# JosefAlbers/Phi-3-Vision-MLX

Hardware: AMD Instinct MI355X
Metric: decode tokens/sec through generate()'s loop (reference-defined; bare graph replays: device_rate) + prefill ms, Phi-3-Vision bf16 1-image VQA (higher is better)
Workload: dtype bf16; 1 GPU; Phi-3-Vision single 336x336 image VQA (BASELINE configs[1]); 17 crops, 2509 image tokens + 22 text tokens, prompt 2531, B=1 per GPU, greedy, EOS suppressed; parallelism=batch-sharded replicas x1, batch_per_gpu=1, tiny=False

## Files before the change

### phi-3-vision-mlx_amd/csrc/p3v_common.h

```cpp
#pragma once
#include <hip/hip_runtime.h>
#include <stdint.h>

#include "../../include/p3v.h"

typedef uint16_t bf16_t;
typedef __attribute__((ext_vector_type(8))) __bf16 bf16x8_t;
typedef __attribute__((ext_vector_type(4))) float f32x4_t;
typedef __attribute__((ext_vector_type(16))) float f32x16_t;
typedef __attribute__((ext_vector_type(4))) uint32_t u32x4_t;
typedef __attribute__((ext_vector_type(2))) uint32_t u32x2_t;

#define P3V_WAVE 64
#define P3V_MAX_DEVICES 64

#define P3V_CHECK_LAUNCH()                                   \
  do {                                                       \
    hipError_t e_ = hipGetLastError();                       \
    if (e_ != hipSuccess) return P3V_ERR_LAUNCH;             \
  } while (0)

__device__ __forceinline__ float bf16_to_f32(bf16_t u) { return __uint_as_float(((uint32_t)u) << 16); }

typedef __attribute__((ext_vector_type(2))) __bf16 bf16x2_t;
// ... 46 lines not shown
__device__ __forceinline__ float rows_sum(float v) {
  float a, b;
  rows_swap32(v, a, b); v = a + b;
  rows_swap16(v, a, b); return a + b;
}

#define P3V_DPP_F32(v, ctrl) __builtin_bit_cast(float, __builtin_amdgcn_update_dpp(0, __builtin_bit_cast(int, v), ctrl, 0xf, 0xf, true))
__device__ __forceinline__ float wave_sum(float v) {
  v += P3V_DPP_F32(v, 0xB1);
  v += P3V_DPP_F32(v, 0x4E);
  v += P3V_DPP_F32(v, 0x124);
  v += P3V_DPP_F32(v, 0x128);
  return rows_sum(v);
}
__device__ __forceinline__ float wave_max(float v) {
  v = fmaxf(v, P3V_DPP_F32(v, 0xB1));
  v = fmaxf(v, P3V_DPP_F32(v, 0x4E));
  v = fmaxf(v, P3V_DPP_F32(v, 0x124));
  v = fmaxf(v, P3V_DPP_F32(v, 0x128));
  return rows_max(v);
}

__device__ __forceinline__ float block_sum(float v, float* red) {
  v = wave_sum(v);
  const int w = threadIdx.x >> 6, nw = blockDim.x >> 6;
  __syncthreads();
  if ((threadIdx.x & 63) == 0) red[w] = v;
  __syncthreads();
  float t = 0.f;
  for (int i = 0; i < nw; ++i) t += red[i];
  return t;
}
__device__ __forceinline__ float block_max(float v, float* red) {
  v = wave_max(v);
  const int w = threadIdx.x >> 6, nw = blockDim.x >> 6;
  __syncthreads();
  if ((threadIdx.x & 63) == 0) red[w] = v;
  __syncthreads();
  float t = -INFINITY;
  for (int i = 0; i < nw; ++i) t = fmaxf(t, red[i]);
  return t;
}

static inline int p3v_cdiv(long a, long b) { return (int)((a + b - 1) / b); }
static inline int p3v_gemv_wpw(int waves, int n_cu, int forced) {
  if (forced == 3 || forced == 4) return forced;
  const float w3 = (float)p3v_cdiv(p3v_cdiv(waves, 3), n_cu) * 3.f * n_cu / (float)waves;
  const float w4 = (float)p3v_cdiv(p3v_cdiv(waves, 4), n_cu) * 4.f * n_cu / (float)waves;
  return w3 < w4 - 0.05f ? 3 : 4;
}

struct P3vTuning {
  int gemm_big_rows;
  int gemm_no_splitk, gemm_splitk_max_m, gemm_splitk_max_s, gemm_splitk_wgs, gemm_128, gemm_persistent;
  int gemm_rows;
  int gemm_no_skinny, gemm_skinny_max_m, gemm_skinny_s, gemm_skinny_tm128;
  int gemm_no_qkv_fuse;
  int gemm_f8_narrow;
  int attn_no_dma, attn_old, attn_pp, attn_il, attn_il_waves, combine_g, kvq_old, q8_old;
  int attn_fo_map_q8;
  int attn_fo_map;
  int gemv_no_mfma, gemv_no_mfma8, gemv_wpc, gemv8_wgs, gemv_variant, gemv_rows, gemv8_min, gemv_mfma8, gemv_f8_wpc, gemv_q4_wpc, gemv_wpw, gemv_q4_rows_wgs, gemv_q4_rows8;
};
const P3vTuning& p3v_tuning();
```

### phi-3-vision-mlx_amd/csrc/p3v_gemm.hip

```cpp
#include <stdlib.h>
#include <string.h>


#include "p3v_gemm_qkv.h"

#define P3V_EPI_QKV 100

#define BM 128
#define BN 128
#define BK 64
#define TILE_BYTES (BM * BK * 2)
#define GEMM_LDS (4 * TILE_BYTES)

typedef const __attribute__((address_space(1))) void* gptr_t;
typedef __attribute__((address_space(3))) void* lptr_t;

struct GemmP {
  const bf16_t* A; const bf16_t* W; void* out; const bf16_t* bias; const void* resid; const bf16_t* pos;
  int M, N, K, lda, ldw, ldo, ppi;
  int kslice;
  QkvP q;
};

__device__ __forceinline__ float gelu_erf(float x) { return 0.5f * x * (1.f + erff(x * 0.70710678118654752f)); }
// ... 204 lines not shown
#pragma unroll
    for (int jp = 0; jp < 2; ++jp) {
      uint32_t pk[2][2];
#pragma unroll
      for (int jj = 0; jj < 2; ++jj) {
        const int j = 2 * jp + jj;
        float v[4];
#pragma unroll
        for (int r = 0; r < 4; ++r) {
          v[r] = acc[i][j][r] + bias[j][r];
          if (EPI == P3V_EPI_BIAS_QGELU) v[r] = v[r] * p3v_sigmoid(1.702f * v[r]);
          else if (EPI == P3V_EPI_BIAS_GELU) v[r] = gelu_erf(v[r]);
        }
        pk[jj][0] = pack_bf16x2(v[0], v[1]), pk[jj][1] = pack_bf16x2(v[2], v[3]);
      }
      u32x4_t w;
#pragma unroll
      for (int k = 0; k < 2; ++k) {
        auto sw = __builtin_amdgcn_permlane16_swap(pk[0][k], pk[1][k], false, false);
        w[k] = sw[0], w[2 + k] = sw[1];
      }
      const int n = n0 + wc * 64 + (2 * jp + (fq & 1)) * 16 + (fq >> 1) * 8;
      if (m < p.M && n < p.N) {
        const size_t o = (size_t)m * p.ldo + n;
        if (EPI == P3V_EPI_RESID_BF16) {
          const u32x4_t rw = *(const u32x4_t*)((const bf16_t*)p.resid + o);
#pragma unroll
          for (int k = 0; k < 4; ++k) w[k] = pack_bf16x2(bf16lo(rw[k]) + bf16lo(w[k]), bf16hi(rw[k]) + bf16hi(w[k]));
        }
        *(u32x4_t*)((bf16_t*)p.out + o) = w;
      }
    }
  }
}

template <int EPI, int ORD>
static int launch_gemm_v(const GemmP& p, hipStream_t s) {
  static bool attr_set = false;
  if (!attr_set) {
    if (hipFuncSetAttribute((const void*)k_gemm<EPI, ORD>, hipFuncAttributeMaxDynamicSharedMemorySize, GEMM_LDS) != hipSuccess)
      return P3V_ERR_HIP;
    attr_set = true;
  }
  const int n_tile = EPI == P3V_EPI_SILU_MUL ? BN / 2 : BN;
  dim3 grid(p3v_cdiv(p.N, n_tile), p3v_cdiv(p.M, BM), p.kslice ? p.K / p.kslice : 1);
  hipLaunchKernelGGL((k_gemm<EPI, ORD>), grid, dim3(256), GEMM_LDS, s, p);
  P3V_CHECK_LAUNCH();
  return P3V_OK;
}

template <int EPI>
static int launch_gemm(const GemmP& p, hipStream_t s) { return launch_gemm_v<EPI, 0>(p, s); }

int p3v_gemm256_try(const p3v_gemm_args_t* a, hipStream_t s);
static int gemm128(const p3v_gemm_args_t* a, hipStream_t s);

static int gemm_big_rows(const p3v_gemm_args_t* a) {
  const int n_big = a->epilogue == P3V_EPI_SILU_MUL ? 128 : 256, n_small = n_big / 2;
  if (a->M < 1024 || a->N % n_big || a->epilogue == P3V_EPI_PATCH) return 0;
  if (const int force = p3v_tuning().gemm_big_rows; force >= 0) return min(force / 256 * 256, a->M);
  const int mt = p3v_cdiv(a->M, 256), nt_big = a->N / n_big, nt_small = p3v_cdiv(a->N, n_small);
  const float big_round = a->K >= 2048 ? 1.0f : 1.0f + 0.25f * (2048 - a->K) / 1024.f;
  float best = 1e30f;
  int best_rows = 0;
  for (int ms = 0; ms <= mt; ++ms) {
    const int rows_big = min(ms * 256, a->M), rows_small = a->M - rows_big;
    const long big = (long)ms * nt_big, small = (long)p3v_cdiv(rows_small, 128) * nt_small;
    float c = (float)((big + 255) / 256) * big_round;
    if (small) {
      const long full = small / 512, rest = small % 512;
      c += 0.675f * full + (rest == 0 ? 0.f : rest <= 256 ? 0.42f : 0.675f);
    }
    if (big && small) c += 0.04f;
    if (c < best - 1e-4f) { best = c; best_rows = rows_big; }
  }
  return best_rows;
}

template <int EPI>
__global__ void __launch_bounds__(256) k_splitk_reduce(const float* __restrict__ part, void* __restrict__ out, const void* __restrict__ resid,
                                                       int M, int N, int ldp, int ldo, int S) {
  constexpr bool SILU = EPI == P3V_EPI_SILU_MUL;
  const int per_row = N / 8;
  const long i = (long)blockIdx.x * 256 + threadIdx.x;
  if (i >= (long)M * per_row) return;
  const int m = (int)(i / per_row), n = (int)(i - (long)m * per_row) * 8;
  float v[8] = {0, 0, 0, 0, 0, 0, 0, 0}, u[8] = {0, 0, 0, 0, 0, 0, 0, 0};
  for (int z = 0; z < S; ++z) {
    const float* pr = part + ((size_t)z * M + m) * ldp + n;
    const float4 a0 = *(const float4*)pr, a1 = *(const float4*)(pr + 4);
    v[0] += a0.x; v[1] += a0.y; v[2] += a0.z; v[3] += a0.w; v[4] += a1.x; v[5] += a1.y; v[6] += a1.z; v[7] += a1.w;
    if (SILU) {
      const float4 b0 = *(const float4*)(pr + N), b1 = *(const float4*)(pr + N + 4);
      u[0] += b0.x; u[1] += b0.y; u[2] += b0.z; u[3] += b0.w; u[4] += b1.x; u[5] += b1.y; u[6] += b1.z; u[7] += b1.w;
    }
  }
  const size_t o = (size_t)m * ldo + n;
  if (SILU) {
#pragma unroll
    for (int e = 0; e < 8; ++e) {
      const float g = bf16_round(v[e]), up = bf16_round(u[e]);
      v[e] = bf16_round(g * bf16_round(1.f / (1.f + __expf(-g)))) * up;
    }
  } else if (EPI == P3V_EPI_RESID_BF16) {
    float r[8];
    load8_bf16((const bf16_t*)resid + o, r);
#pragma unroll
    for (int e = 0; e < 8; ++e) v[e] = r[e] + bf16_round(v[e]);
  }
  store8_bf16((bf16_t*)out + o, v);
}

__global__ void __launch_bounds__(384) k_splitk_reduce_norm(const float* __restrict__ part, bf16_t* __restrict__ out, const bf16_t* __restrict__ resid,
                                                            const u32x4_t* __restrict__ norm_w, u32x4_t* __restrict__ normed, int M, int N,
                                                            int ldo, int S, float inv_h, float eps) {
  __shared__ float ps[6 * 4][64];
  __shared__ float r_sh;
  const int row = blockIdx.x, c = threadIdx.x, lane = c & 63, wv = c >> 6, chunks = N / 8;
  u32x4_t v = {0u, 0u, 0u, 0u}, g = {0u, 0u, 0u, 0u};
  if (c < chunks) {
    float acc[8] = {0, 0, 0, 0, 0, 0, 0, 0};
    for (int z = 0; z < S; ++z) {
      const float* pr = part + ((size_t)z * M + row) * N + c * 8;
      const float4 a0 = *(const float4*)pr, a1 = *(const float4*)(pr + 4);
      acc[0] += a0.x; acc[1] += a0.y; acc[2] += a0.z; acc[3] += a0.w; acc[4] += a1.x; acc[5] += a1.y; acc[6] += a1.z; acc[7] += a1.w;
    }
    const size_t o = (size_t)row * ldo + c * 8;
    float r[8];
    load8_bf16(resid + o, r);
// ... 76 lines not shown
}

int p3v_splitk_reduce(const float* part, const p3v_gemm_args_t* a, int S, hipStream_t s) {
  const bool silu = a->epilogue == P3V_EPI_SILU_MUL;
  const int w_rows = silu ? 2 * a->N : a->N;
  const long items = (long)a->M * (a->N / 8);
  const dim3 grid((unsigned)p3v_cdiv(items, 256));
  if (silu) hipLaunchKernelGGL(k_splitk_reduce<P3V_EPI_SILU_MUL>, grid, dim3(256), 0, s, part, a->out, a->resid, a->M, a->N, w_rows, a->ldo, S);
  else if (a->epilogue == P3V_EPI_RESID_BF16)
    hipLaunchKernelGGL(k_splitk_reduce<P3V_EPI_RESID_BF16>, grid, dim3(256), 0, s, part, a->out, a->resid, a->M, a->N, w_rows, a->ldo, S);
  else hipLaunchKernelGGL(k_splitk_reduce<P3V_EPI_NONE>, grid, dim3(256), 0, s, part, a->out, a->resid, a->M, a->N, w_rows, a->ldo, S);
  P3V_CHECK_LAUNCH();
  return P3V_OK;
}

static int gemm_splitk(const p3v_gemm_args_t* a, hipStream_t s) {
  const bool silu = a->epilogue == P3V_EPI_SILU_MUL;
  const int S = splitk_slices(a->M, a->N, a->K, a->epilogue);
  if (S == 1) return P3V_ERR_UNSUPPORTED;
  const int w_rows = silu ? 2 * a->N : a->N;
  if (!a->ws || a->ws_bytes < (int64_t)S * a->M * w_rows * 4) return P3V_ERR_UNSUPPORTED;
  if ((uintptr_t)a->ws & 15) return P3V_ERR_ARG;
  float* part = (float*)a->ws;
  GemmP p = {a->A, a->W, part, nullptr, nullptr, nullptr, a->M, w_rows, a->K, a->lda, a->ldw, w_rows, 0, a->K / S, {}};
  const int rc = launch_gemm<P3V_EPI_F32>(p, s);
  if (rc != P3V_OK) return rc;
  return p3v_splitk_reduce(part, a, S, s);
}

extern "C" int p3v_gemm(const p3v_gemm_args_t* a, void* stream) {
  if (!a || !a->A || !a->W || !a->out) return P3V_ERR_ARG;
  if (a->M < 0 || a->N <= 0 || a->K <= 0 || a->K % BK || a->N % 8 || a->ldo % 8) return P3V_ERR_ARG;
  if (a->lda < a->K || a->ldw < a->K || a->lda % 8 || a->ldw % 8) return P3V_ERR_ARG;
  if (((uintptr_t)a->A | (uintptr_t)a->W | (uintptr_t)a->out | (uintptr_t)a->resid | (uintptr_t)a->bias | (uintptr_t)a->pos) & 15)
    return P3V_ERR_ARG;
  if ((a->epilogue == P3V_EPI_BIAS_RESID_F32 || a->epilogue == P3V_EPI_RESID_BF16) && !a->resid) return P3V_ERR_ARG;
  if (a->epilogue == P3V_EPI_PATCH && (!a->pos || a->patches_per_img <= 0)) return P3V_ERR_ARG;
  if (a->epilogue < 0 || a->epilogue > P3V_EPI_F32) return P3V_ERR_ARG;
  if (a->M == 0) return P3V_OK;
  {
    const size_t w_rows = (size_t)a->N * (a->epilogue == P3V_EPI_SILU_MUL ? 2 : 1);
    if ((size_t)a->M * a->lda * 2 >= (1ull << 32) || w_rows * a->ldw * 2 >= (1ull << 32)) return P3V_ERR_UNSUPPORTED;
  }
  hipStream_t s = (hipStream_t)stream;
  if (!a->bias) {
    const int rc = p3v_gemm_skinny_try(a, s);
    if (rc != P3V_ERR_UNSUPPORTED) return rc;
  }
  {
    const int rc = gemm_splitk(a, s);
    if (rc != P3V_ERR_UNSUPPORTED) return rc;
  }
  const bool big_tiles = !p3v_tuning().gemm_128;
  const int rows_big = big_tiles ? gemm_big_rows(a) : 0;
  if (rows_big > 0) {
    p3v_gemm_args_t top = *a;
    top.M = rows_big;
    const int rc = p3v_gemm256_try(&top, s);
    if (rc == P3V_OK && rows_big < a->M) {
      const bool f32_out = a->epilogue == P3V_EPI_BIAS_RESID_F32 || a->epilogue == P3V_EPI_F32;
      const size_t out_row = (size_t)a->ldo * (f32_out ? 4 : 2);
      p3v_gemm_args_t rest = *a;
      rest.M = a->M - rows_big;
      rest.A = a->A + (size_t)rows_big * a->lda;
      rest.out = (char*)a->out + rows_big * out_row;
      if (a->resid) rest.resid = (const char*)a->resid + rows_big * out_row;
      return gemm128(&rest, s);
    }
    if (rc != P3V_ERR_UNSUPPORTED) return rc;
  }
  return gemm128(a, s);
}

static int gemm128(const p3v_gemm_args_t* a, hipStream_t s) {
  const GemmP p = {a->A, a->W, a->out, a->bias, a->resid, a->pos,
                   a->M, a->N, a->K, a->lda, a->ldw, a->ldo, a->patches_per_img, 0, {}};
  switch (a->epilogue) {
    case P3V_EPI_NONE: return launch_gemm<P3V_EPI_NONE>(p, s);
    case P3V_EPI_BIAS: return launch_gemm<P3V_EPI_BIAS>(p, s);
    case P3V_EPI_BIAS_QGELU: return launch_gemm<P3V_EPI_BIAS_QGELU>(p, s);
    case P3V_EPI_BIAS_GELU: return launch_gemm<P3V_EPI_BIAS_GELU>(p, s);
    case P3V_EPI_BIAS_RESID_F32: return launch_gemm<P3V_EPI_BIAS_RESID_F32>(p, s);
    case P3V_EPI_RESID_BF16: return launch_gemm<P3V_EPI_RESID_BF16>(p, s);
    case P3V_EPI_SILU_MUL: return launch_gemm<P3V_EPI_SILU_MUL>(p, s);
    case P3V_EPI_PATCH: return launch_gemm<P3V_EPI_PATCH>(p, s);
    case P3V_EPI_F32: return launch_gemm<P3V_EPI_F32>(p, s);
    default: return P3V_ERR_ARG;
  }
}

int p3v_gemm256_qkv(const p3v_gemm_args_t* a, const QkvP& q, hipStream_t s);
int p3v_gemm_skinny_qkv(const p3v_gemm_args_t* a, const QkvP& q, hipStream_t s);

extern "C" int p3v_gemm_qkv(const p3v_gemm_args_t* a, const p3v_qkv_split_t* sp, void* stream) {
  if (!a || !sp || !a->A || !a->W || !sp->q_out || !sp->k_dst || !sp->v_dst || (!sp->cos_t) != (!sp->sin_t)) return P3V_ERR_ARG;
  if (a->epilogue != P3V_EPI_NONE && a->epilogue != P3V_EPI_BIAS) return P3V_ERR_ARG;
  if (a->epilogue == P3V_EPI_BIAS && !a->bias) return P3V_ERR_ARG;
  const int nh = sp->n_heads, nkv = sp->n_kv, hd = sp->hd, half = hd / 2;
  if (sp->B <= 0 || sp->L <= 0 || nh <= 0 || nkv <= 0 || hd <= 0 || sp->tab_div <= 0 || !(sp->q_scale > 0.f)) return P3V_ERR_ARG;
  if (a->M != sp->B * sp->L || a->N != (nh + 2 * nkv) * hd || a->K % BK || a->lda < a->K || a->ldw < a->K || a->lda % 8 || a->ldw % 8) return P3V_ERR_ARG;
  if (((uintptr_t)a->A | (uintptr_t)a->W | (uintptr_t)a->bias | (uintptr_t)sp->q_out | (uintptr_t)sp->k_dst | (uintptr_t)sp->v_dst |
       (uintptr_t)sp->cos_t | (uintptr_t)sp->sin_t) & 15)
    return P3V_ERR_ARG;
  const int dpos0 = sp->dst_off_is_past ? sp->past : 0;
  if (hd % 32 || half % 16 || dpos0 % 8 || sp->dst_t % 8 || p3v_tuning().gemm_no_qkv_fuse) return P3V_ERR_UNSUPPORTED;
  if ((size_t)a->M * a->lda * 2 >= (1ull << 32) || (size_t)a->N * a->ldw * 2 >= (1ull << 32)) return P3V_ERR_UNSUPPORTED;
  hipStream_t s = (hipStream_t)stream;
  QkvP q = {sp->cos_t, sp->sin_t, sp->q_out, sp->k_dst, sp->v_dst, sp->L, nh, nkv, hd, sp->past, dpos0, sp->dst_t, sp->tab_t, sp->tab_div, 0,
            sp->q_scale};
  if (a->M < 1024) return p3v_gemm_skinny_qkv(a, q, s);
  if ((nh * hd) % BN || (nkv * hd) % BN || p3v_tuning().gemm_128) return P3V_ERR_UNSUPPORTED;
// ... 18 lines not shown
```

### phi-3-vision-mlx_amd/csrc/p3v_gemm256.hip

```cpp
#include <stdlib.h>

#include "p3v_gemm256_epi.h"

#define BUF_BYTES (4 * HALF_BYTES)
#define GEMM256_LDS (2 * BUF_BYTES)

struct Tile256 {
  int m0, n0; int a_off[2][2], b_off[2][2]; __amdgpu_buffer_rsrc_t rs_a;
  int swapped, is_k, row0;
};

#ifdef P3V_G256_DEBUG
__device__ unsigned long long p3v_g256dbg[8 * 64 * 8];
#define G_S(k) do { __builtin_amdgcn_sched_barrier(0); asm volatile("s_memtime %0" : "=s"(g_s[k])); __builtin_amdgcn_sched_barrier(0); } while (0)
#define G_FLUSH(it) do { if (blockIdx.x == P3V_G256_DEBUG && (threadIdx.x & 63) == 0 && (it) < 64) { for (int k_ = 0; k_ < 8; ++k_) p3v_g256dbg[((threadIdx.x >> 6) * 64 + (it)) * 8 + k_] = g_s[k_]; } } while (0)
extern "C" int p3v_g256dbg_read(unsigned long long* out) {
  return hipMemcpyFromSymbol(out, HIP_SYMBOL(p3v_g256dbg), sizeof(unsigned long long) * 8 * 64 * 8) == hipSuccess ? 0 : -1;
}
#else
#define G_S(k) do { } while (0)
#define G_FLUSH(it) do { } while (0)
#endif
template <int EPI, int SCHED = 0x50, int ORDER = 0>
__global__ void __launch_bounds__(512, 1) k_gemm256(Gemm256P p) {
  constexpr bool SILU = EPI == P3V_EPI_SILU_MUL, QKV = EPI == P3V_EPI_QKV;
  extern __shared__ __attribute__((aligned(16))) unsigned char smem[];
  const int tid = threadIdx.x, lane = tid & 63, wave = __builtin_amdgcn_readfirstlane(tid >> 6);
  const int wr = wave >> 2, wc = wave & 3;
  constexpr int n_out_tile = SILU ? TN / 2 : TN;
  const int gx = (p.N + n_out_tile - 1) / n_out_tile, gy = (p.M + TM - 1) / TM, nwg = gx * gy;
  const int nq_t = QKV ? p.q.nh * p.q.hd / TN : 0, nk_t = QKV ? p.q.nkv * p.q.hd / TN : 0;

  using Tile = Tile256;
  const int srow = tid >> 3, schunk = tid & 7;
  auto make_tile = [&](int wid, Tile& t) {
    const int q = nwg >> 3, r = nwg & 7, xcd = wid & 7, loc = wid >> 3;
    const int id = (xcd < r ? xcd * (q + 1) : r * (q + 1) + (xcd - r) * q) + loc;
    constexpr int BAND = 4;
    const int band = id / (BAND * gx), in_band = id % (BAND * gx);
    const int rows = min(BAND, gy - band * BAND);
    const int m_t = band * BAND + in_band % rows, n_t = in_band / rows;
    t.m0 = m_t * TM, t.n0 = n_t * n_out_tile;
    t.swapped = t.is_k = t.row0 = 0;
    if (QKV) {
      t.swapped = n_t >= nq_t + nk_t;
      t.is_k = !t.swapped && n_t >= nq_t;
      t.row0 = t.swapped ? (p.q.nh + p.q.nkv) * p.q.hd : t.is_k ? p.q.nh * p.q.hd : 0;
      t.n0 = (n_t - (t.swapped ? nq_t + nk_t : t.is_k ? nq_t : 0)) * TN;
    }
#pragma unroll
    for (int h = 0; h < 2; ++h)
#pragma unroll
      for (int qq = 0; qq < 2; ++qq) {
        const int rr = h * 128 + qq * 64 + srow;
        const int sw = (schunk ^ (rr & 7)) * 8;
        const int ar = min(t.m0 + rr, p.M - 1) - t.m0;
        int br;
        if (SILU) {
          const int wcol = rr >> 6, ni = (rr & 63) >> 4, c = rr & 15;
          br = min(t.n0 + wcol * 32 + (ni & 1) * 16 + c, p.N - 1) + (ni >> 1) * p.N;
        } else if (QKV) {
          br = qkv_pair_row(p.q, t.row0, t.n0 >> 1, rr);
        } else {
          br = min(t.n0 + rr, p.N - 1);
        }
        if (QKV && t.swapped) {
          t.a_off[h][qq] = (rr * p.ldw + sw) * 2;
          t.b_off[h][qq] = (int)(((unsigned)(t.m0 + ar) * (unsigned)p.lda + (unsigned)sw) * 2u);
        } else {
          t.a_off[h][qq] = (ar * p.lda + sw) * 2;
          t.b_off[h][qq] = (int)(((unsigned)br * (unsigned)p.ldw + (unsigned)sw) * 2u);
        }
      }
    t.rs_a = QKV && t.swapped ? __builtin_amdgcn_make_buffer_rsrc((void*)(p.W + (size_t)(t.row0 + t.n0) * p.ldw), 0, 0xffffffff, 0x00020000)
                              : __builtin_amdgcn_make_buffer_rsrc((void*)(p.A + (size_t)t.m0 * p.lda), 0, 0xffffffff, 0x00020000);
  };
  const __amdgpu_buffer_rsrc_t rs_w = __builtin_amdgcn_make_buffer_rsrc((void*)p.W, 0, 0xffffffff, 0x00020000);
  const __amdgpu_buffer_rsrc_t rs_x = __builtin_amdgcn_make_buffer_rsrc((void*)p.A, 0, 0xffffffff, 0x00020000);
  auto dma_half = [&](const Tile& t, int which, int kt, int buf) {
    unsigned char* base = smem + buf * BUF_BYTES + which * HALF_BYTES + wave * 1024;
    const int h = which & 1;
#pragma unroll
    for (int q = 0; q < 2; ++q) {
      const __amdgpu_buffer_rsrc_t rs = which < 2 ? t.rs_a : (QKV && t.swapped) ? rs_x : rs_w;
      const int vo = which < 2 ? t.a_off[h][q] : t.b_off[h][q];
      __builtin_amdgcn_raw_ptr_buffer_load_lds(rs, (lptr_t)(base + q * 8192), 16, vo, kt * (TK * 2), 0, 0);
    }
  };

  const int frow = lane & 15, fchunk = lane >> 4;
  const int nk = p.K / TK;
  int wid = blockIdx.x;
  if (wid >= nwg) return;
  Tile cur_t;
  make_tile(wid, cur_t);
#pragma unroll
  for (int w4 = 0; w4 < 4; ++w4) dma_half(cur_t, w4, 0, 0);
  int gk = 0;
  bool landed = false;
  for (;;) {
  const int m0 = cur_t.m0, n0 = cur_t.n0;
  const bool has_next = wid + (int)gridDim.x < nwg;
  f32x4_t acc[8][4];
#pragma unroll
  for (int i = 0; i < 8; ++i)
#pragma unroll
    for (int j = 0; j < 4; ++j) acc[i][j] = (f32x4_t){0.f, 0.f, 0.f, 0.f};

#ifdef P3V_G256_DEBUG
  unsigned long long g_s[8] = {0, 0, 0, 0, 0, 0, 0, 0};
#endif
  for (int kt = 0; kt < nk; ++kt, ++gk) {
    G_S(0);
    if (!(kt == 0 && landed)) asm volatile("s_waitcnt vmcnt(0)" ::: "memory");
    G_S(1);
    __builtin_amdgcn_s_barrier();
    G_S(2);
    const bool last = kt + 1 == nk;
    const bool more = !last || has_next;
    const int nb = (gk + 1) & 1;
    const unsigned char* ta = smem + (gk & 1) * BUF_BYTES + wr * HALF_BYTES;
    const unsigned char* tb = smem + (gk & 1) * BUF_BYTES + (2 + (wc >> 1)) * HALF_BYTES + (wc & 1) * 64 * 128;
    bf16x8_t af[4][2], af1[4][2], bf0[2][2], bf1[2][2];
    auto read_a_to = [&](int sub, bf16x8_t (&dst)[4][2]) {
#pragma unroll
      for (int i = 0; i < 4; ++i)
#pragma unroll
        for (int kk = 0; kk < 2; ++kk) {
          const int r = sub * 64 + i * 16 + frow;
          dst[i][kk] = *(const bf16x8_t*)(ta + r * 128 + (((kk * 4 + fchunk) ^ (r & 7)) << 4));
        }
    };
    auto read_a = [&](int sub) { read_a_to(sub, af); };
    auto read_b = [&](int sub, bf16x8_t (&bf)[2][2]) {
#pragma unroll
      for (int j = 0; j < 2; ++j)
#pragma unroll
        for (int kk = 0; kk < 2; ++kk) {
          const int r = sub * 32 + j * 16 + frow;
          bf[j][kk] = *(const bf16x8_t*)(tb + r * 128 + (((kk * 4 + fchunk) ^ (r & 7)) << 4));
        }
    };
    auto quad_from = [&](int asub, int bsub, bf16x8_t (&a)[4][2], bf16x8_t (&bf)[2][2]) {
      __builtin_amdgcn_s_setprio(1);
#pragma unroll
      for (int kk = 0; kk < 2; ++kk)
#pragma unroll
        for (int i = 0; i < 4; ++i)
#pragma unroll
          for (int j = 0; j < 2; ++j)
            acc[asub * 4 + i][bsub * 2 + j] =
                __builtin_amdgcn_mfma_f32_16x16x32_bf16(bf[j][kk], a[i][kk], acc[asub * 4 + i][bsub * 2 + j], 0, 0, 0);
      __builtin_amdgcn_s_setprio(0);
    };
    auto quad = [&](int asub, int bsub, bf16x8_t (&bf)[2][2]) { quad_from(asub, bsub, af, bf); };
    auto dma_phase = [&](int ph) {
      if (more) {
#pragma unroll
        for (int h = 0; h < 4; ++h)
          if (((SCHED >> (2 * h)) & 3) == ph) {
            if (!last) dma_half(cur_t, h, kt + 1, nb);
            else {
              Tile nt;
              make_tile(wid + gridDim.x, nt);
              dma_half(nt, h, 0, nb);
            }
          }
      }
    };
    if (ORDER == 2) {
      read_b(0, bf0);
      read_a_to(0, af);
      dma_phase(0);
      read_b(1, bf1);
      __builtin_amdgcn_sched_barrier(0);
      G_S(3);
      quad_from(0, 0, af, bf0);
      __builtin_amdgcn_sched_barrier(0);
      G_S(4);
      read_a_to(1, af1);
      dma_phase(1);
      __builtin_amdgcn_sched_barrier(0);
      G_S(5);
      quad_from(0, 1, af, bf1);
      __builtin_amdgcn_sched_barrier(0);
      G_S(6);
      quad_from(1, 1, af1, bf1);
      quad_from(1, 0, af1, bf0);
      G_S(7);
      G_FLUSH(kt);
      continue;
    }
    if (ORDER == 0) dma_phase(0);
    read_b(0, bf0);
    read_a(0);
    if (ORDER == 1) dma_phase(0);
    quad(0, 0, bf0);
    if (ORDER == 0) dma_phase(1);
    read_b(1, bf1);
    if (ORDER == 1) dma_phase(1);
    quad(0, 1, bf1);
    if (ORDER == 0) dma_phase(2);
    read_a(1);
    if (ORDER == 1) dma_phase(2);
    quad(1, 1, bf1);
    dma_phase(3);
    quad(1, 0, bf0);
  }

  if (has_next) {
    asm volatile("s_waitcnt vmcnt(0)" ::: "memory");
    landed = true;
  }
  if constexpr (QKV) {
    if (!cur_t.swapped) qkv_epilogue_rot<8>(p.q, acc, p.bias, cur_t.is_k, cur_t.row0, (n0 >> 1) + wc * 32, m0 + wr * 128, p.M, lane);
    else qkv_epilogue_vt<8>(p.q, acc, p.bias ? p.bias + cur_t.row0 : nullptr, n0 + wr * 128, m0 + wc * 64, p.M, lane);
  } else {
    gemm256_epilogue<EPI>(p, acc, m0, n0, wr, wc, lane);
  }
  if (!has_next) break;
  wid += gridDim.x;
  make_tile(wid, cur_t);
  }
}

template <int EPI, int SCHED, int ORDER>
static int launch_gemm256_v(const Gemm256P& p, hipStream_t s) {
  static bool attr_set = false;
  if (!attr_set) {
    if (hipFuncSetAttribute((const void*)k_gemm256<EPI, SCHED, ORDER>, hipFuncAttributeMaxDynamicSharedMemorySize, GEMM256_LDS) != hipSuccess)
      return P3V_ERR_HIP;
    attr_set = true;
  }
  const int n_tile = EPI == P3V_EPI_SILU_MUL ? TN / 2 : TN;
  static int n_cu = 0;
  if (!n_cu) {
    int dev = 0;
    hipDeviceProp_t pr;
    if (hipGetDevice(&dev) != hipSuccess || hipGetDeviceProperties(&pr, dev) != hipSuccess) return P3V_ERR_HIP;
    n_cu = pr.multiProcessorCount / 8 * 8;
  }
  const int tiles = p3v_cdiv(p.N, n_tile) * p3v_cdiv(p.M, TM);
  const int persist = p3v_tuning().gemm_persistent;
  dim3 grid(persist ? min(tiles, n_cu) : tiles);
  hipLaunchKernelGGL((k_gemm256<EPI, SCHED, ORDER>), grid, dim3(512), GEMM256_LDS, s, p);
  P3V_CHECK_LAUNCH();
  return P3V_OK;
}

template <int EPI>
static int launch_gemm256(const Gemm256P& p, hipStream_t s) { return launch_gemm256_v<EPI, 0x50, 2>(p, s); }

int p3v_gemm256_qkv(const p3v_gemm_args_t* a, const QkvP& q, hipStream_t s) {
  if (a->N % TN || a->K % TK || (q.nh * q.hd) % TN || (q.nkv * q.hd) % TN) return P3V_ERR_UNSUPPORTED;
  if ((size_t)a->N * a->ldw * 2 >= ((size_t)1 << 32) || (size_t)a->M * a->lda * 2 >= ((size_t)1 << 32)) return P3V_ERR_UNSUPPORTED;
  const Gemm256P p = {a->A, a->W, nullptr, a->bias, nullptr, a->M, a->N, a->K, a->lda, a->ldw, 0, q};
  return launch_gemm256<P3V_EPI_QKV>(p, s);
}

int p3v_gemm256_try(const p3v_gemm_args_t* a, hipStream_t s) {
  const int n_tile = a->epilogue == P3V_EPI_SILU_MUL ? TN / 2 : TN;
  if (a->N % n_tile || a->K % TK || a->epilogue == P3V_EPI_PATCH) return P3V_ERR_UNSUPPORTED;
  const size_t w_rows = (size_t)a->N * (a->epilogue == P3V_EPI_SILU_MUL ? 2 : 1);
  if (w_rows * a->ldw * 2 >= ((size_t)1 << 32) || (size_t)256 * a->lda * 2 >= ((size_t)1 << 31)) return P3V_ERR_UNSUPPORTED;
  const Gemm256P p = {a->A, a->W, a->out, a->bias, a->resid, a->M, a->N, a->K, a->lda, a->ldw, a->ldo, {}};
  switch (a->epilogue) {
    case P3V_EPI_NONE: return launch_gemm256<P3V_EPI_NONE>(p, s);
    case P3V_EPI_BIAS: return launch_gemm256<P3V_EPI_BIAS>(p, s);
    case P3V_EPI_BIAS_QGELU: return launch_gemm256<P3V_EPI_BIAS_QGELU>(p, s);
    case P3V_EPI_BIAS_GELU: return launch_gemm256<P3V_EPI_BIAS_GELU>(p, s);
    case P3V_EPI_BIAS_RESID_F32: return launch_gemm256<P3V_EPI_BIAS_RESID_F32>(p, s);
    case P3V_EPI_RESID_BF16: return launch_gemm256<P3V_EPI_RESID_BF16>(p, s);
    case P3V_EPI_SILU_MUL: return launch_gemm256<P3V_EPI_SILU_MUL>(p, s);
    case P3V_EPI_F32: return launch_gemm256<P3V_EPI_F32>(p, s);
    default: return P3V_ERR_UNSUPPORTED;
  }
}
```

### phi-3-vision-mlx_amd/csrc/p3v_gemm256_epi.h

```cpp
#pragma once
#include "p3v_gemm_qkv.h"

#define P3V_EPI_QKV 100

#define TM 256
#define TN 256
#define TK 64
#define HALF_BYTES (128 * TK * 2)

typedef const __attribute__((address_space(1))) void* gptr_t;
typedef __attribute__((address_space(3))) void* lptr_t;

struct Gemm256P {
  const bf16_t* A; const bf16_t* W; void* out; const bf16_t* bias; const void* resid;
  int M, N, K, lda, ldw, ldo;
  QkvP q;
};

__device__ __forceinline__ float gelu_erf2(float x) { return 0.5f * x * (1.f + erff(x * 0.70710678118654752f)); }

template <int EPI>
__device__ __forceinline__ void gemm256_epilogue(const Gemm256P& p, f32x4_t (&acc)[8][4], int m0, int n0, int wr, int wc, int lane) {
  constexpr bool SILU = EPI == P3V_EPI_SILU_MUL;
  const int fc = lane & 15, fq = lane >> 4;
  const int mrow0 = m0 + wr * 128 + fc;
#if defined(P3V_G256_ABL) && P3V_G256_ABL == 3
#pragma unroll
  for (int i = 0; i < 8; ++i)
#pragma unroll
    for (int j = 0; j < 4; ++j) asm volatile("" :: "v"(acc[i][j]));
#else
  if (SILU) {
    const int n = n0 + wc * 32 + (fq & 1) * 16 + (fq >> 1) * 8;
#pragma unroll
    for (int i = 0; i < 8; ++i) {
      uint32_t pk[2][2];
#pragma unroll
      for (int j = 0; j < 2; ++j) {
        float o4[4];
#pragma unroll
        for (int r = 0; r < 4; ++r) {
          const float g = bf16_round(acc[i][j][r]), u = bf16_round(acc[i][2 + j][r]);
          o4[r] = bf16_round(g * bf16_round(1.f / (1.f + __expf(-g)))) * u;
        }
        pk[j][0] = pack_bf16x2(o4[0], o4[1]), pk[j][1] = pack_bf16x2(o4[2], o4[3]);
      }
      u32x4_t w;
#pragma unroll
      for (int k = 0; k < 2; ++k) {
        auto sw = __builtin_amdgcn_permlane16_swap(pk[0][k], pk[1][k], false, false);
        w[k] = sw[0], w[2 + k] = sw[1];
      }
      const int m = mrow0 + i * 16;
      if (m < p.M && n < p.N) *(u32x4_t*)((bf16_t*)p.out + (size_t)m * p.ldo + n) = w;
    }
  } else if (EPI == P3V_EPI_BIAS_RESID_F32 || EPI == P3V_EPI_F32) {
    float bias[4][4];
#pragma unroll
    for (int j = 0; j < 4; ++j) {
      const int n = n0 + wc * 64 + j * 16 + fq * 4;
      u32x2_t bw = {0u, 0u};
      if (p.bias && n < p.N) bw = *(const u32x2_t*)(p.bias + n);
      bias[j][0] = bf16lo(bw[0]), bias[j][1] = bf16hi(bw[0]), bias[j][2] = bf16lo(bw[1]), bias[j][3] = bf16hi(bw[1]);
    }
#pragma unroll
    for (int i = 0; i < 8; ++i) {
      const int m = mrow0 + i * 16;
#pragma unroll
      for (int j = 0; j < 4; ++j) {
        const int n = n0 + wc * 64 + j * 16 + fq * 4;
        if (m < p.M && n < p.N) {
          const size_t o = (size_t)m * p.ldo + n;
          float4 v = make_float4(acc[i][j][0] + bias[j][0], acc[i][j][1] + bias[j][1], acc[i][j][2] + bias[j][2], acc[i][j][3] + bias[j][3]);
          if (EPI == P3V_EPI_BIAS_RESID_F32) {
            const float4 r4 = *(const float4*)((const float*)p.resid + o);
            v.x += r4.x, v.y += r4.y, v.z += r4.z, v.w += r4.w;
          }
          *(float4*)((float*)p.out + o) = v;
        }
      }
    }
  } else {
    float bias[4][4];
#pragma unroll
    for (int j = 0; j < 4; ++j) {
      const int n = n0 + wc * 64 + j * 16 + fq * 4;
      u32x2_t bw = {0u, 0u};
      if (p.bias && n < p.N) bw = *(const u32x2_t*)(p.bias + n);
      bias[j][0] = bf16lo(bw[0]), bias[j][1] = bf16hi(bw[0]), bias[j][2] = bf16lo(bw[1]), bias[j][3] = bf16hi(bw[1]);
    }
#pragma unroll
    for (int i = 0; i < 8; ++i) {
      const int m = mrow0 + i * 16;
#pragma unroll
      for (int jp = 0; jp < 2; ++jp) {
        uint32_t pk[2][2];
#pragma unroll
        for (int jj = 0; jj < 2; ++jj) {
          const int j = 2 * jp + jj;
          float v[4];
#pragma unroll
          for (int r = 0; r < 4; ++r) {
            v[r] = acc[i][j][r] + bias[j][r];
            if (EPI == P3V_EPI_BIAS_QGELU) v[r] = v[r] * p3v_sigmoid(1.702f * v[r]);
            else if (EPI == P3V_EPI_BIAS_GELU) v[r] = gelu_erf2(v[r]);
          }
          pk[jj][0] = pack_bf16x2(v[0], v[1]), pk[jj][1] = pack_bf16x2(v[2], v[3]);
        }
        u32x4_t w;
#pragma unroll
        for (int k = 0; k < 2; ++k) {
          auto sw = __builtin_amdgcn_permlane16_swap(pk[0][k], pk[1][k], false, false);
          w[k] = sw[0], w[2 + k] = sw[1];
        }
        const int n = n0 + wc * 64 + (2 * jp + (fq & 1)) * 16 + (fq >> 1) * 8;
        if (m < p.M && n < p.N) {
          const size_t o = (size_t)m * p.ldo + n;
          if (EPI == P3V_EPI_RESID_BF16) {
            const u32x4_t rw = *(const u32x4_t*)((const bf16_t*)p.resid + o);
#pragma unroll
            for (int k = 0; k < 4; ++k) w[k] = pack_bf16x2(bf16lo(rw[k]) + bf16lo(w[k]), bf16hi(rw[k]) + bf16hi(w[k]));
          }
#if defined(P3V_G256_ABL) && P3V_G256_ABL == 1
          asm volatile("" :: "v"(w));
#else
          *(u32x4_t*)((bf16_t*)p.out + o) = w;
#endif
        }
      }
    }
  }
#endif
}
```

### phi-3-vision-mlx_amd/csrc/p3v_runtime.hip

```cpp
#include <ctype.h>
#include <stdlib.h>
#include <string.h>

#include <mutex>

#include "p3v_common.h"

extern "C" int p3v_version(void) { return P3V_VERSION; }

extern "C" const char* p3v_strerror(int code) {
  switch (code) {
    case P3V_OK: return "ok";
    case P3V_ERR_ARG: return "invalid argument (shape, alignment or null pointer)";
    case P3V_ERR_LAUNCH: return "kernel launch failed";
    case P3V_ERR_UNSUPPORTED: return "unsupported combination";
    case P3V_ERR_HIP: return "HIP runtime call failed";
    default: return "unknown error";
  }
}

namespace {
struct Knob { const char* name; int P3vTuning::*field; int dflt; };
const Knob kKnobs[] = {
    {"gemm_big_rows", &P3vTuning::gemm_big_rows, -1},       {"gemm_no_splitk", &P3vTuning::gemm_no_splitk, 0},
    {"gemm_splitk_max_m", &P3vTuning::gemm_splitk_max_m, 1024}, {"gemm_splitk_max_s", &P3vTuning::gemm_splitk_max_s, 8},
    {"gemm_splitk_wgs", &P3vTuning::gemm_splitk_wgs, 256},  {"gemm_128", &P3vTuning::gemm_128, 0},
    {"gemm_persistent", &P3vTuning::gemm_persistent, 1},     {"gemm_no_qkv_fuse", &P3vTuning::gemm_no_qkv_fuse, 0},
    {"gemm_f8_narrow", &P3vTuning::gemm_f8_narrow, -1},     {"attn_no_dma", &P3vTuning::attn_no_dma, 0},
    {"attn_old", &P3vTuning::attn_old, 0},                  {"attn_pp", &P3vTuning::attn_pp, -1},
    {"attn_il", &P3vTuning::attn_il, -1},                   {"attn_il_waves", &P3vTuning::attn_il_waves, -1},
                      {"combine_g", &P3vTuning::combine_g, -1},
    {"kvq_old", &P3vTuning::kvq_old, 0},                    {"q8_old", &P3vTuning::q8_old, 0},
    {"gemv_no_mfma", &P3vTuning::gemv_no_mfma, 0},          {"gemv_no_mfma8", &P3vTuning::gemv_no_mfma8, 0},
    {"gemv_wpc", &P3vTuning::gemv_wpc, 8},                  {"gemv8_wgs", &P3vTuning::gemv8_wgs, 256},
    {"gemv_variant", &P3vTuning::gemv_variant, 3},          {"gemv_rows", &P3vTuning::gemv_rows, 1},
    {"gemv8_min", &P3vTuning::gemv8_min, 2},                {"gemv_mfma8", &P3vTuning::gemv_mfma8, 1},
    {"gemv_f8_wpc", &P3vTuning::gemv_f8_wpc, 16},           {"gemv_q4_wpc", &P3vTuning::gemv_q4_wpc, 8},
    {"gemv_wpw", &P3vTuning::gemv_wpw, 0},                  {"gemv_q4_rows_wgs", &P3vTuning::gemv_q4_rows_wgs, 256},
    {"gemv_q4_rows8", &P3vTuning::gemv_q4_rows8, 1},
    {"gemm_no_skinny", &P3vTuning::gemm_no_skinny, 0},      {"gemm_skinny_max_m", &P3vTuning::gemm_skinny_max_m, 256},
    {"gemm_skinny_s", &P3vTuning::gemm_skinny_s, 0},            {"gemm_skinny_tm128", &P3vTuning::gemm_skinny_tm128, 0},
    {"gemm_rows", &P3vTuning::gemm_rows, 1},
    {"attn_fo_map", &P3vTuning::attn_fo_map, 2},              {"attn_fo_map_q8", &P3vTuning::attn_fo_map_q8, 0},
};
P3vTuning g_tuning;
std::once_flag g_tuning_once;
void tuning_init() {
  for (const Knob& k : kKnobs) {
    char env[64] = "P3V_";
    size_t n = 4;
    for (const char* c = k.name; *c && n + 1 < sizeof(env); ++c) env[n++] = (char)toupper((unsigned char)*c);
    env[n] = 0;
    const char* e = getenv(env);
    g_tuning.*(k.field) = !e ? k.dflt : !strcmp(e, "auto") ? -1 : (*e == 0 ? 1 : atoi(e));
  }
}
}

const P3vTuning& p3v_tuning() {
  std::call_once(g_tuning_once, tuning_init);
  return g_tuning;
}

extern "C" int p3v_set_tuning(const char* name, int value) {
  if (!name) return P3V_ERR_ARG;
  std::call_once(g_tuning_once, tuning_init);
  for (const Knob& k : kKnobs)
    if (!strcmp(k.name, name)) { g_tuning.*(k.field) = value; return P3V_OK; }
  return P3V_ERR_ARG;
}

extern "C" int p3v_get_tuning(const char* name, int* value) {
  if (!name || !value) return P3V_ERR_ARG;
  std::call_once(g_tuning_once, tuning_init);
  for (const Knob& k : kKnobs)
    if (!strcmp(k.name, name)) { *value = g_tuning.*(k.field); return P3V_OK; }
  return P3V_ERR_ARG;
}

extern "C" int p3v_device_props(int device, p3v_props_t* out) {
  if (!out) return P3V_ERR_ARG;
  hipDeviceProp_t pr;
  if (hipGetDeviceProperties(&pr, device) != hipSuccess) return P3V_ERR_HIP;
  memset(out, 0, sizeof(*out));
  out->cu_count = pr.multiProcessorCount;
  out->lds_per_cu = (int)pr.maxSharedMemoryPerMultiProcessor;
  out->wave_size = pr.warpSize;
  out->clock_khz = pr.clockRate;
  out->mem_clock_khz = pr.memoryClockRate;
  out->mem_bus_bits = pr.memoryBusWidth;
  out->hbm_bytes = (int64_t)pr.totalGlobalMem;
  strncpy(out->arch, pr.gcnArchName, sizeof(out->arch) - 1);
  return P3V_OK;
}

// ... 45 lines not shown
```

Measured before the change: 534.4 tokens/s.

## Add 128-row half-tile variant of 256 GEMM selected by wave-quantization cost

```diff
diff --git a/phi-3-vision-mlx_amd/csrc/p3v_common.h b/phi-3-vision-mlx_amd/csrc/p3v_common.h
--- a/phi-3-vision-mlx_amd/csrc/p3v_common.h
+++ b/phi-3-vision-mlx_amd/csrc/p3v_common.h
@@ -122,6 +122,7 @@
 
 struct P3vTuning {
   int gemm_big_rows;
+  int gemm_half;
   int gemm_no_splitk, gemm_splitk_max_m, gemm_splitk_max_s, gemm_splitk_wgs, gemm_128, gemm_persistent;
   int gemm_rows;
   int gemm_no_skinny, gemm_skinny_max_m, gemm_skinny_s, gemm_skinny_tm128;
diff --git a/phi-3-vision-mlx_amd/csrc/p3v_gemm.hip b/phi-3-vision-mlx_amd/csrc/p3v_gemm.hip
--- a/phi-3-vision-mlx_amd/csrc/p3v_gemm.hip
+++ b/phi-3-vision-mlx_amd/csrc/p3v_gemm.hip
@@ -280,10 +280,10 @@
 template <int EPI>
 static int launch_gemm(const GemmP& p, hipStream_t s) { return launch_gemm_v<EPI, 0>(p, s); }
 
-int p3v_gemm256_try(const p3v_gemm_args_t* a, hipStream_t s);
+int p3v_gemm256_try(const p3v_gemm_args_t* a, bool half, hipStream_t s);
 static int gemm128(const p3v_gemm_args_t* a, hipStream_t s);
 
-static int gemm_big_rows(const p3v_gemm_args_t* a) {
+static int gemm_big_rows(const p3v_gemm_args_t* a, float* cost = nullptr) {
   const int n_big = a->epilogue == P3V_EPI_SILU_MUL ? 128 : 256, n_small = n_big / 2;
   if (a->M < 1024 || a->N % n_big || a->epilogue == P3V_EPI_PATCH) return 0;
   if (const int force = p3v_tuning().gemm_big_rows; force >= 0) return min(force / 256 * 256, a->M);
@@ -302,7 +302,19 @@
     if (big && small) c += 0.04f;
     if (c < best - 1e-4f) { best = c; best_rows = rows_big; }
   }
+  if (cost) *cost = best;
   return best_rows;
+}
+
+#define GEMM_HALF_ROUND 0.55f
+static bool gemm_half_tiles(const p3v_gemm_args_t* a, float packed_cost) {
+  const int half = p3v_tuning().gemm_half;
+  if (half == 0 || a->N % 256 || a->epilogue == P3V_EPI_PATCH) return false;
+  if (half > 0) return true;
+  if (a->M < 1024 || a->epilogue == P3V_EPI_SILU_MUL || p3v_tuning().gemm_big_rows >= 0) return false;
+  const float big_round = a->K >= 2048 ? 1.0f : 1.0f + 0.25f * (2048 - a->K) / 1024.f;
+  const long tiles = (long)p3v_cdiv(a->M, 128) * (a->N / 256);
+  return (float)((tiles + 255) / 256) * GEMM_HALF_ROUND * big_round < packed_cost - 1e-4f;
 }
 
 template <int EPI>
@@ -485,11 +497,16 @@
     if (rc != P3V_ERR_UNSUPPORTED) return rc;
   }
   const bool big_tiles = !p3v_tuning().gemm_128;
-  const int rows_big = big_tiles ? gemm_big_rows(a) : 0;
+  float packed_cost = 0.f;
+  const int rows_big = big_tiles ? gemm_big_rows(a, &packed_cost) : 0;
+  if (big_tiles && gemm_half_tiles(a, packed_cost)) {
+    const int rc = p3v_gemm256_try(a, true, s);
+    if (rc != P3V_ERR_UNSUPPORTED) return rc;
+  }
   if (rows_big > 0) {
     p3v_gemm_args_t top = *a;
     top.M = rows_big;
-    const int rc = p3v_gemm256_try(&top, s);
+    const int rc = p3v_gemm256_try(&top, false, s);
     if (rc == P3V_OK && rows_big < a->M) {
       const bool f32_out = a->epilogue == P3V_EPI_BIAS_RESID_F32 || a->epilogue == P3V_EPI_F32;
       const size_t out_row = (size_t)a->ldo * (f32_out ? 4 : 2);
diff --git a/phi-3-vision-mlx_amd/csrc/p3v_gemm256.hip b/phi-3-vision-mlx_amd/csrc/p3v_gemm256.hip
--- a/phi-3-vision-mlx_amd/csrc/p3v_gemm256.hip
+++ b/phi-3-vision-mlx_amd/csrc/p3v_gemm256.hip
@@ -21,14 +21,16 @@
 #define G_S(k) do { } while (0)
 #define G_FLUSH(it) do { } while (0)
 #endif
-template <int EPI, int SCHED = 0x50, int ORDER = 0>
+template <int EPI, int SCHED = 0x50, int ORDER = 0, bool HALF = false>
 __global__ void __launch_bounds__(512, 1) k_gemm256(Gemm256P p) {
   constexpr bool SILU = EPI == P3V_EPI_SILU_MUL, QKV = EPI == P3V_EPI_QKV;
+  static_assert(!HALF || (ORDER == 2 && !QKV), "128-row tiles: the pipelined K loop, plain epilogues");
+  constexpr int TMR = HALF ? TM / 2 : TM;
   extern __shared__ __attribute__((aligned(16))) unsigned char smem[];
   const int tid = threadIdx.x, lane = tid & 63, wave = __builtin_amdgcn_readfirstlane(tid >> 6);
   const int wr = wave >> 2, wc = wave & 3;
   constexpr int n_out_tile = SILU ? TN / 2 : TN;
-  const int gx = (p.N + n_out_tile - 1) / n_out_tile, gy = (p.M + TM - 1) / TM, nwg = gx * gy;
+  const int gx = (p.N + n_out_tile - 1) / n_out_tile, gy = (p.M + TMR - 1) / TMR, nwg = gx * gy;
   const int nq_t = QKV ? p.q.nh * p.q.hd / TN : 0, nk_t = QKV ? p.q.nkv * p.q.hd / TN : 0;
 
   using Tile = Tile256;
@@ -40,7 +42,7 @@
     const int band = id / (BAND * gx), in_band = id % (BAND * gx);
     const int rows = min(BAND, gy - band * BAND);
     const int m_t = band * BAND + in_band % rows, n_t = in_band / rows;
-    t.m0 = m_t * TM, t.n0 = n_t * n_out_tile;
+    t.m0 = m_t * TMR, t.n0 = n_t * n_out_tile;
     t.swapped = t.is_k = t.row0 = 0;
     if (QKV) {
       t.swapped = n_t >= nq_t + nk_t;
@@ -95,7 +97,8 @@
   Tile cur_t;
   make_tile(wid, cur_t);
 #pragma unroll
-  for (int w4 = 0; w4 < 4; ++w4) dma_half(cur_t, w4, 0, 0);
+  for (int w4 = 0; w4 < 4; ++w4)
+    if (!(HALF && w4 == 1)) dma_half(cur_t, w4, 0, 0);
   int gk = 0;
   bool landed = false;
   for (;;) {
@@ -119,7 +122,7 @@
     const bool last = kt + 1 == nk;
     const bool more = !last || has_next;
     const int nb = (gk + 1) & 1;
-    const unsigned char* ta = smem + (gk & 1) * BUF_BYTES + wr * HALF_BYTES;
+    const unsigned char* ta = smem + (gk & 1) * BUF_BYTES + (HALF ? 0 : wr) * HALF_BYTES;
     const unsigned char* tb = smem + (gk & 1) * BUF_BYTES + (2 + (wc >> 1)) * HALF_BYTES + (wc & 1) * 64 * 128;
     bf16x8_t af[4][2], af1[4][2], bf0[2][2], bf1[2][2];
     auto read_a_to = [&](int sub, bf16x8_t (&dst)[4][2]) {
@@ -158,7 +161,7 @@
       if (more) {
 #pragma unroll
         for (int h = 0; h < 4; ++h)
-          if (((SCHED >> (2 * h)) & 3) == ph) {
+          if (((SCHED >> (2 * h)) & 3) == ph && !(HALF && h == 1)) {
             if (!last) dma_half(cur_t, h, kt + 1, nb);
             else {
               Tile nt;
@@ -168,6 +171,19 @@
           }
       }
     };
+    if constexpr (HALF) {
+      read_b(0, bf0);
+      read_a_to(wr, af);
+      dma_phase(0);
+      read_b(1, bf1);
+      __builtin_amdgcn_sched_barrier(0);
+      quad_from(0, 0, af, bf0);
+      __builtin_amdgcn_sched_barrier(0);
+      dma_phase(1);
+      __builtin_amdgcn_sched_barrier(0);
+      quad_from(0, 1, af, bf1);
+      continue;
+    }
     if (ORDER == 2) {
       read_b(0, bf0);
       read_a_to(0, af);
@@ -216,7 +232,7 @@
     if (!cur_t.swapped) qkv_epilogue_rot<8>(p.q, acc, p.bias, cur_t.is_k, cur_t.row0, (n0 >> 1) + wc * 32, m0 + wr * 128, p.M, lane);
     else qkv_epilogue_vt<8>(p.q, acc, p.bias ? p.bias + cur_t.row0 : nullptr, n0 + wr * 128, m0 + wc * 64, p.M, lane);
   } else {
-    gemm256_epilogue<EPI>(p, acc, m0, n0, wr, wc, lane);
+    gemm256_epilogue<EPI, HALF ? 4 : 8>(p, acc, m0, n0, wr, wc, lane);
   }
   if (!has_next) break;
   wid += gridDim.x;
@@ -224,11 +240,11 @@
   }
 }
 
-template <int EPI, int SCHED, int ORDER>
+template <int EPI, int SCHED, int ORDER, bool HALF = false>
 static int launch_gemm256_v(const Gemm256P& p, hipStream_t s) {
   static bool attr_set = false;
   if (!attr_set) {
-    if (hipFuncSetAttribute((const void*)k_gemm256<EPI, SCHED, ORDER>, hipFuncAttributeMaxDynamicSharedMemorySize, GEMM256_LDS) != hipSuccess)
+    if (hipFuncSetAttribute((const void*)k_gemm256<EPI, SCHED, ORDER, HALF>, hipFuncAttributeMaxDynamicSharedMemorySize, GEMM256_LDS) != hipSuccess)
       return P3V_ERR_HIP;
     attr_set = true;
   }
@@ -240,39 +256,41 @@
     if (hipGetDevice(&dev) != hipSuccess || hipGetDeviceProperties(&pr, dev) != hipSuccess) return P3V_ERR_HIP;
     n_cu = pr.multiProcessorCount / 8 * 8;
   }
-  const int tiles = p3v_cdiv(p.N, n_tile) * p3v_cdiv(p.M, TM);
+  const int tiles = p3v_cdiv(p.N, n_tile) * p3v_cdiv(p.M, HALF ? TM / 2 : TM);
   const int persist = p3v_tuning().gemm_persistent;
   dim3 grid(persist ? min(tiles, n_cu) : tiles);
-  hipLaunchKernelGGL((k_gemm256<EPI, SCHED, ORDER>), grid, dim3(512), GEMM256_LDS, s, p);
+  hipLaunchKernelGGL((k_gemm256<EPI, SCHED, ORDER, HALF>), grid, dim3(512), GEMM256_LDS, s, p);
   P3V_CHECK_LAUNCH();
   return P3V_OK;
 }
 
 template <int EPI>
-static int launch_gemm256(const Gemm256P& p, hipStream_t s) { return launch_gemm256_v<EPI, 0x50, 2>(p, s); }
+static int launch_gemm256(const Gemm256P& p, bool half, hipStream_t s) {
+  return half ? launch_gemm256_v<EPI, 0x50, 2, true>(p, s) : launch_gemm256_v<EPI, 0x50, 2>(p, s);
+}
 
 int p3v_gemm256_qkv(const p3v_gemm_args_t* a, const QkvP& q, hipStream_t s) {
   if (a->N % TN || a->K % TK || (q.nh * q.hd) % TN || (q.nkv * q.hd) % TN) return P3V_ERR_UNSUPPORTED;
   if ((size_t)a->N * a->ldw * 2 >= ((size_t)1 << 32) || (size_t)a->M * a->lda * 2 >= ((size_t)1 << 32)) return P3V_ERR_UNSUPPORTED;
   const Gemm256P p = {a->A, a->W, nullptr, a->bias, nullptr, a->M, a->N, a->K, a->lda, a->ldw, 0, q};
-  return launch_gemm256<P3V_EPI_QKV>(p, s);
-}
-
-int p3v_gemm256_try(const p3v_gemm_args_t* a, hipStream_t s) {
+  return launch_gemm256_v<P3V_EPI_QKV, 0x50, 2>(p, s);
+}
+
+int p3v_gemm256_try(const p3v_gemm_args_t* a, bool half, hipStream_t s) {
   const int n_tile = a->epilogue == P3V_EPI_SILU_MUL ? TN / 2 : TN;
   if (a->N % n_tile || a->K % TK || a->epilogue == P3V_EPI_PATCH) return P3V_ERR_UNSUPPORTED;
   const size_t w_rows = (size_t)a->N * (a->epilogue == P3V_EPI_SILU_MUL ? 2 : 1);
   if (w_rows * a->ldw * 2 >= ((size_t)1 << 32) || (size_t)256 * a->lda * 2 >= ((size_t)1 << 31)) return P3V_ERR_UNSUPPORTED;
   const Gemm256P p = {a->A, a->W, a->out, a->bias, a->resid, a->M, a->N, a->K, a->lda, a->ldw, a->ldo, {}};
   switch (a->epilogue) {
-    case P3V_EPI_NONE: return launch_gemm256<P3V_EPI_NONE>(p, s);
-    case P3V_EPI_BIAS: return launch_gemm256<P3V_EPI_BIAS>(p, s);
-    case P3V_EPI_BIAS_QGELU: return launch_gemm256<P3V_EPI_BIAS_QGELU>(p, s);
-    case P3V_EPI_BIAS_GELU: return launch_gemm256<P3V_EPI_BIAS_GELU>(p, s);
-    case P3V_EPI_BIAS_RESID_F32: return launch_gemm256<P3V_EPI_BIAS_RESID_F32>(p, s);
-    case P3V_EPI_RESID_BF16: return launch_gemm256<P3V_EPI_RESID_BF16>(p, s);
-    case P3V_EPI_SILU_MUL: return launch_gemm256<P3V_EPI_SILU_MUL>(p, s);
-    case P3V_EPI_F32: return launch_gemm256<P3V_EPI_F32>(p, s);
+    case P3V_EPI_NONE: return launch_gemm256<P3V_EPI_NONE>(p, half, s);
+    case P3V_EPI_BIAS: return launch_gemm256<P3V_EPI_BIAS>(p, half, s);
+    case P3V_EPI_BIAS_QGELU: return launch_gemm256<P3V_EPI_BIAS_QGELU>(p, half, s);
+    case P3V_EPI_BIAS_GELU: return launch_gemm256<P3V_EPI_BIAS_GELU>(p, half, s);
+    case P3V_EPI_BIAS_RESID_F32: return launch_gemm256<P3V_EPI_BIAS_RESID_F32>(p, half, s);
+    case P3V_EPI_RESID_BF16: return launch_gemm256<P3V_EPI_RESID_BF16>(p, half, s);
+    case P3V_EPI_SILU_MUL: return launch_gemm256<P3V_EPI_SILU_MUL>(p, half, s);
+    case P3V_EPI_F32: return launch_gemm256<P3V_EPI_F32>(p, half, s);
     default: return P3V_ERR_UNSUPPORTED;
   }
 }
diff --git a/phi-3-vision-mlx_amd/csrc/p3v_gemm256_epi.h b/phi-3-vision-mlx_amd/csrc/p3v_gemm256_epi.h
--- a/phi-3-vision-mlx_amd/csrc/p3v_gemm256_epi.h
+++ b/phi-3-vision-mlx_amd/csrc/p3v_gemm256_epi.h
@@ -19,21 +19,21 @@
 
 __device__ __forceinline__ float gelu_erf2(float x) { return 0.5f * x * (1.f + erff(x * 0.70710678118654752f)); }
 
-template <int EPI>
+template <int EPI, int NI = 8>
 __device__ __forceinline__ void gemm256_epilogue(const Gemm256P& p, f32x4_t (&acc)[8][4], int m0, int n0, int wr, int wc, int lane) {
   constexpr bool SILU = EPI == P3V_EPI_SILU_MUL;
   const int fc = lane & 15, fq = lane >> 4;
-  const int mrow0 = m0 + wr * 128 + fc;
+  const int mrow0 = m0 + wr * NI * 16 + fc;
 #if defined(P3V_G256_ABL) && P3V_G256_ABL == 3
 #pragma unroll
-  for (int i = 0; i < 8; ++i)
+  for (int i = 0; i < NI; ++i)
 #pragma unroll
     for (int j = 0; j < 4; ++j) asm volatile("" :: "v"(acc[i][j]));
 #else
   if (SILU) {
     const int n = n0 + wc * 32 + (fq & 1) * 16 + (fq >> 1) * 8;
 #pragma unroll
-    for (int i = 0; i < 8; ++i) {
+    for (int i = 0; i < NI; ++i) {
       uint32_t pk[2][2];
 #pragma unroll
       for (int j = 0; j < 2; ++j) {
@@ -64,7 +64,7 @@
       bias[j][0] = bf16lo(bw[0]), bias[j][1] = bf16hi(bw[0]), bias[j][2] = bf16lo(bw[1]), bias[j][3] = bf16hi(bw[1]);
     }
 #pragma unroll
-    for (int i = 0; i < 8; ++i) {
+    for (int i = 0; i < NI; ++i) {
       const int m = mrow0 + i * 16;
 #pragma unroll
       for (int j = 0; j < 4; ++j) {
@@ -90,7 +90,7 @@
       bias[j][0] = bf16lo(bw[0]), bias[j][1] = bf16hi(bw[0]), bias[j][2] = bf16lo(bw[1]), bias[j][3] = bf16hi(bw[1]);
     }
 #pragma unroll
-    for (int i = 0; i < 8; ++i) {
+    for (int i = 0; i < NI; ++i) {
       const int m = mrow0 + i * 16;
 #pragma unroll
       for (int jp = 0; jp < 2; ++jp) {
diff --git a/phi-3-vision-mlx_amd/csrc/p3v_runtime.hip b/phi-3-vision-mlx_amd/csrc/p3v_runtime.hip
--- a/phi-3-vision-mlx_amd/csrc/p3v_runtime.hip
+++ b/phi-3-vision-mlx_amd/csrc/p3v_runtime.hip
@@ -40,7 +40,7 @@
     {"gemv_q4_rows8", &P3vTuning::gemv_q4_rows8, 1},
     {"gemm_no_skinny", &P3vTuning::gemm_no_skinny, 0},      {"gemm_skinny_max_m", &P3vTuning::gemm_skinny_max_m, 256},
     {"gemm_skinny_s", &P3vTuning::gemm_skinny_s, 0},            {"gemm_skinny_tm128", &P3vTuning::gemm_skinny_tm128, 0},
-    {"gemm_rows", &P3vTuning::gemm_rows, 1},
+    {"gemm_rows", &P3vTuning::gemm_rows, 1},                {"gemm_half", &P3vTuning::gemm_half, -1},
     {"attn_fo_map", &P3vTuning::attn_fo_map, 2},              {"attn_fo_map_q8", &P3vTuning::attn_fo_map_q8, 0},
 };
 P3vTuning g_tuning;
```

After: 531.5 tokens/s, median of 3. No clear change (-0.5%).
